# lxtGH/Video-K-Net

Hardware: AMD Instinct MI355X
Metric: frames/sec (S=3, N=100, 1024x2048) (higher is better)
Workload: dtype f32; 1 GPU; cfg2 video_knet_s3_r50: VideoKernelIterHead S=3, N=100 proposals + 17 stuff = 117 kernels, C=256, 1024x2048 frame -> 128x256 stride-8 features, ffn tracking link, x4 bilinear upsample of the final logits; streams_per_gpu=1, parallelism=frame-sharded dp1, x_storage=fp32

## Files before the change

include/vkn.h:

```cpp
#ifndef VKN_H
#define VKN_H
#include <stddef.h>
#include <stdint.h>

#ifdef __cplusplus
extern "C" {
#endif

#define VKN_VERSION 0x000600

#define VKN_OK 0
#define VKN_E_ARG (-1)
#define VKN_E_SHAPE (-2)
#define VKN_E_WORKSPACE (-3)
#define VKN_E_LAUNCH (-4)
#define VKN_E_ALIGN (-5)
#define VKN_E_RANGE (-6)

#define VKN_STATUS_RANGE 1u

#define VKN_FLAG_REF_KERNELS 1u
#define VKN_FLAG_EXACT_GEMM 2u
#define VKN_FLAG_LOGITS_HANDOFF 4u
#define VKN_FLAG_BITS_HANDOFF 16u
#define VKN_X_F32 0
#define VKN_X_F16 1
#define VKN_X_BF16 2
#define VKN_FLAG_X_F16 64u
#define VKN_FLAG_X_BF16 128u
#define VKN_FLAG_CHAIN_LAUNCHES 256u
#define VKN_FLAG_CHAIN_PERSISTENT 512u
#define VKN_FLAG_JOIN_EARLY 32768u
#define VKN_FLAG_LINK_RESERVE 262144u
#define VKN_FLAG_LINK_NO_RESERVE 524288u
#define VKN_FLAG_SCALED_F16 16384u
#define VKN_FLAG_CHAIN_BF16X3 65536u
#define VKN_FLAG_CHAIN_KSPLIT 8192u
#define VKN_FLAG_SERIAL_LINK 32u
#define VKN_FLAG_CLIP_LINK 8u

#define VKN_FLAG_INIT_SEPARATE 131072u
#define VKN_FLAG_PHASE_A 1024u
#define VKN_FLAG_PHASE_B 2048u
#define VKN_FLAG_PHASE_C 4096u
#define VKN_FLAG_PHASE_MASK (VKN_FLAG_PHASE_A | VKN_FLAG_PHASE_B | VKN_FLAG_PHASE_C)

#define VKN_MAX_FCS 4

typedef struct VknDims {
    int B;
    int N;
    int C;
    int H, W;
    int heads;
    int ff;
    int ncls;
    int n_cls_fcs, n_mask_fcs;
    float thr_logit;
    float ln_eps;
} VknDims;

typedef struct VknStageWeights {
    const float *ft_w, *ft_b, *ft_wT;
    const float *dyn_w, *dyn_b;
    const float *inp_w, *inp_b;
    const float *ig_w, *ig_b, *ug_w, *ug_b;
    const float *norm_in_w, *norm_in_b;
    const float *norm_out_w, *norm_out_b;
    const float *inorm_in_w, *inorm_in_b;
// ... 346 lines not shown
```

video-k-net_amd/csrc/vkn_api.hip:

```cpp
#include "../../include/vkn.h"
#include "../../include/vkn_decode.h"
#include "vkn_common.h"
#include "vkn_launch.h"

namespace {

struct Carver {
    char* base;
    size_t off;
    template <class T>
    T* take(size_t n) {
        off = (off + 255) & ~(size_t)255;
        T* p = base ? reinterpret_cast<T*>(base + off) : nullptr;
        off += n * sizeof(T);
        return p;
    }
};

inline bool aligned16(const void* p) { return (reinterpret_cast<uintptr_t>(p) & 15) == 0; }
inline int npt_of(int N) { return (N + 31) / 32 * 32; }

struct StageWs {
    float *part, *cntp, *xraw, *cnt, *xfeat, *params, *inputf, *ig, *ug, *f, *obj1, *qkv, *ao, *obj2, *h, *partial, *t1, *t2,
        *maskfeat, *kb, *kern32, *lq, *lkv, *lobj, *lupd, *lf;
// ... 144 lines not shown
    const int rt = (M + 31) / 32, ktiles = K / 32;
    int ks = 256 / (rt > 0 ? rt : 1);
    if (ks > 16) ks = 16;
    if (ks > ktiles) ks = ktiles;
    if (ks < 1) ks = 1;
    return ks;
}

size_t carve_stage(const VknDims* d, char* base, StageWs* s) {
    Carver c{base, 0};
    const size_t B = d->B, N = d->N, C = d->C, P = (size_t)d->H * d->W, M = B * N, FF = d->ff;
    const size_t G = vkn_gather_groups(d->B, (int)P), NPT = npt_of(d->N);
    s->status = c.take<int>(64);
    s->part = c.take<float>(B * G * NPT * C);
    s->cntp = c.take<float>(B * G * NPT);
    s->xraw = c.take<float>(M * C);
    s->cnt = c.take<float>(M);
    s->xfeat = c.take<float>(M * C);
    s->params = c.take<float>(M * 2 * C);
    s->inputf = c.take<float>(M * 2 * C);
    s->ig = c.take<float>(M * 2 * C);
    s->ug = c.take<float>(M * C);
    s->f = c.take<float>(M * C);
    s->obj1 = c.take<float>(M * C);
    s->qkv = c.take<float>(M * 3 * C);
    s->ao = c.take<float>(M * C);
    s->obj2 = c.take<float>(M * C);
    s->h = c.take<float>(M * FF);
    {
        const size_t ks = (size_t)ffn_ksplit((int)M, (int)FF), hs = (size_t)ffn_hsplit((int)M, (int)FF);
        const size_t ks1 = (size_t)ffn_ksplit((int)N, (int)FF), hs1 = (size_t)ffn_hsplit((int)N, (int)FF);
        const size_t k4 = 4;
        const size_t a = (ks > hs ? (ks > k4 ? ks : k4) : (hs > k4 ? hs : k4)) * M * C, b1 = (ks1 > hs1 ? (ks1 > k4 ? ks1 : k4) : (hs1 > k4 ? hs1 : k4)) * N * C;
        s->partial = c.take<float>(a > b1 ? a : b1);
    }
    s->t1 = c.take<float>(M * C);
    s->t2 = c.take<float>(M * C);
    s->maskfeat = c.take<float>(M * C);
    s->kb = c.take<float>(M);
    s->kern32 = c.take<float>(M * C);
    s->lq = c.take<float>(M * C);
    s->lkv = c.take<float>(M * 2 * C);
    s->lobj = c.take<float>(M * C);
    s->lupd = c.take<float>(M * C);
    s->lf = c.take<float>(M * C);
    s->kfh = c.take<_Float16>(B * NPT * C);
    s->kfl = c.take<_Float16>(B * NPT * C);
    return (c.off + 255) & ~(size_t)255;
}

int stage_ws(const VknDims* d, void* ws, size_t ws_bytes, StageWs* s) {
    if (!ws || ws_bytes < carve_stage(d, nullptr, s) || !aligned16(ws)) return VKN_E_WORKSPACE;
    carve_stage(d, static_cast<char*>(ws), s);
    return VKN_OK;
}

struct GatherWs { float *part, *cntp, *cnt; };
size_t carve_gather(int B, int N, int C, int P, char* base, GatherWs* g) {
    const size_t G = vkn_gather_groups(B, P), NPT = npt_of(N);
    Carver c{base, 0};
    g->part = c.take<float>((size_t)B * G * NPT * C);
    g->cntp = c.take<float>((size_t)B * G * NPT);
    g->cnt = c.take<float>((size_t)B * N);
    return (c.off + 255) & ~(size_t)255;
}
size_t carve_planes(int B, int N, int C, char* base, _Float16** kfh, _Float16** kfl) {
    Carver c{base, 0};
// ... 190 lines not shown
        const long long q = grid * 3 / 4;
        return (int)(q > full ? full : (q < d->B ? d->B : q));
    }
    if (mode != 1 || !persistent_chain || d->B < VKN_LINK_RESERVE_MIN_FRAMES || xdt_of(flags) != 0) return 0;
    return grid == VKN_DECODE_CUS ? full : 0;
}

inline int persistent_min_row_tiles(const PrepW& pw, unsigned flags) {
    return (!(flags & VKN_FLAG_CHAIN_BF16X3) && pw.h2_scale && pw.h2[VKN_H2_DYNFT]) ? 22 : 64;
}
inline unsigned pw_off(const VknStageWeights* w, const void* p) {
    return (unsigned)(static_cast<const char*>(p) - static_cast<const char*>(w->prepared));
}
inline bool chain_weights_ok(const PrepW& pw, bool have_cls) {
    return pw.dynft && pw.dyn && pw.dec && pw.inp && pw.ig && pw.ug && pw.fc && pw.attn_in && pw.attn_out && pw.ffn1 && pw.ffn2 &&
           pw.cls_fc[0] && pw.mask_fc[0] && (!have_cls || pw.fc_cls);
}
inline bool chain_stage_ok(const VknDims* d, const VknStageWeights* w, const PrepW& pw, bool have_cls) {
    return chain_shape_ok(d) && w->prepared && w->prepared_bytes < (1ull << 31) && chain_weights_ok(pw, have_cls) && w->ffn1_w &&
           w->cls_ln_w[0] && w->mask_ln_w[0];
}
bool chain_fast_ok(const VknDims* d, const VknStageWeights* w, const PrepW& pw, unsigned flags, bool have_cls) {
    if (flags & (VKN_FLAG_CHAIN_LAUNCHES | VKN_FLAG_EXACT_GEMM)) return false;
    if (vkn_dbg_env("VKN_CHAIN_LAUNCHES", 0)) return false;
    if (!(flags & VKN_FLAG_CHAIN_PERSISTENT) && !vkn_dbg_env("VKN_CHAIN_PERSISTENT", 0) &&
        (d->B * d->N + 31) / 32 < persistent_min_row_tiles(pw, flags))
        return false;
    return pw.chain_consts && chain_stage_ok(d, w, pw, have_cls);
}
inline bool chain_h2(const PrepW& pw, unsigned flags, bool have_cls) {
    return !(flags & VKN_FLAG_CHAIN_BF16X3) && pw.h2_scale && pw.h2[VKN_H2_DYNFT] && pw.h2[VKN_H2_DEC] && (!have_cls || pw.h2[VKN_H2_FCCLS]);
}

int run_chain_fast(const VknDims* d, const VknStageWeights* w, const PrepW& pw, const float* a0, bool a0_raw, const float* cnt,
                   const float* obj_in, float* obj_out, float* cls_logits, bool cls_sigmoid, float* kern32_out, const StageWs& s,
                   hipStream_t st, bool h2 = false) {
    const int M = d->B * d->N, C = d->C;
    VknChainA a{};
    a.a0 = a0; a.obj_in = obj_in; a.rowscale = a0_raw ? cnt : nullptr;
    a.wbase = w->prepared; a.wbytes = w->prepared_bytes;
    if (h2) {
        a.off_dyn = pw_off(w, pw.h2[a0_raw ? VKN_H2_DYNFT : VKN_H2_DYN]);
        a.off_inp = pw_off(w, pw.h2[VKN_H2_INP]); a.off_ig = pw_off(w, pw.h2[VKN_H2_IG]); a.off_ug = pw_off(w, pw.h2[VKN_H2_UG]);
        a.off_fc = pw_off(w, pw.h2[VKN_H2_FC]); a.off_in = pw_off(w, pw.h2[VKN_H2_IN]);
    } else {
        a.off_dyn = pw_off(w, a0_raw ? pw.dynft : pw.dyn);
        a.off_inp = pw_off(w, pw.inp); a.off_ig = pw_off(w, pw.ig); a.off_ug = pw_off(w, pw.ug); a.off_fc = pw_off(w, pw.fc);
        a.off_in = pw_off(w, pw.attn_in);
    }
    a.consts = pw.chain_consts;
    a.eps = d->ln_eps; a.M = M; a.obj1 = s.obj1; a.qkv = s.qkv; a.status = s.status;
    VKN_TRY(h2 ? vkn_launch_chain_a_h2(a, st) : vkn_launch_chain_a(a, st));
    VKN_TRY(vkn_launch_attn(s.qkv, 3 * C, s.qkv + C, s.qkv + 2 * C, 3 * C, s.ao, C, d->B, d->N, d->N, d->heads, C / d->heads, st));
    VknChainC c{};
    c.ao = s.ao; c.obj1 = s.obj1; c.wbase = w->prepared; c.wbytes = w->prepared_bytes;
    if (h2) {
        c.off_out = pw_off(w, pw.h2[VKN_H2_OUT]); c.off_ffn1 = pw_off(w, pw.h2[VKN_H2_FFN1]); c.off_ffn2 = pw_off(w, pw.h2[VKN_H2_FFN2]);
        c.off_clsfc = pw_off(w, pw.h2[VKN_H2_CLSFC]); c.off_maskfc = pw_off(w, pw.h2[VKN_H2_MASKFC]);
        c.off_fccls = pw.h2[VKN_H2_FCCLS] ? pw_off(w, pw.h2[VKN_H2_FCCLS]) : 0u; c.off_dec = pw_off(w, pw.h2[VKN_H2_DEC]);
    } else {
        c.off_out = pw_off(w, pw.attn_out); c.off_ffn1 = pw_off(w, pw.ffn1); c.off_ffn2 = pw_off(w, pw.ffn2);
        c.off_clsfc = pw_off(w, pw.cls_fc[0]); c.off_maskfc = pw_off(w, pw.mask_fc[0]);
        c.off_fccls = pw.fc_cls ? pw_off(w, pw.fc_cls) : 0u; c.off_dec = pw_off(w, pw.dec);
    }
    c.consts = pw.chain_consts; c.kb0 = pw.kb0;
    c.ff = d->ff; c.ncls = d->ncls; c.cls_sigmoid = cls_sigmoid ? 1 : 0; c.eps = d->ln_eps; c.M = M;
    c.obj_out = obj_out; c.cls_out = cls_logits; c.kb_out = s.kb;
    if (kern32_out) c.kern_out = kern32_out;
    else { c.plane_hi = s.kfh; c.plane_lo = s.kfl; }
    c.rows_per_frame = d->N; c.NPT = npt_of(d->N); c.status = s.status;
    return h2 ? vkn_launch_chain_c_h2(c, st) : vkn_launch_chain_c(c, st);
}

#define VKN_KS_MAX_ROW_TILES 16
inline bool ks_width_ok(const VknDims* d) {
    return chain_width_ok(d) && (d->ff % 512 == 0 || d->ff <= 1024);
}
bool chain_ks_ok(const VknDims* d, const VknStageWeights* w, const PrepW& pw, unsigned flags, bool have_cls) {
    if (flags & (VKN_FLAG_CHAIN_LAUNCHES | VKN_FLAG_CHAIN_PERSISTENT | VKN_FLAG_EXACT_GEMM)) return false;
    if (vkn_dbg_env("VKN_CHAIN_LAUNCHES", 0) || vkn_dbg_env("VKN_CHAIN_PERSISTENT", 0) || !vkn_dbg_env("VKN_CHAIN_KSPLIT", 1)) return false;
    if (!(flags & VKN_FLAG_CHAIN_KSPLIT) && (d->B * d->N + 31) / 32 > VKN_KS_MAX_ROW_TILES) return false;
    if (!ks_width_ok(d) || !chain_stage_ok(d, w, pw, have_cls)) return false;
    const void* v16[] = {w->inorm_in_w, w->inorm_in_b, w->norm_in_w, w->norm_in_b, w->norm_out_w, w->norm_out_b, w->inorm_out_w, w->inorm_out_b,
                         w->fc_norm_w, w->fc_norm_b, w->attn_norm_w, w->attn_norm_b, w->ffn_norm_w, w->ffn_norm_b, w->ffn2_b,
                         w->cls_ln_w[0], w->cls_ln_b[0], w->mask_ln_w[0], w->mask_ln_b[0], pw.dvec};
    for (const void* p : v16)
        if (!p || !aligned16(p)) return false;
    return true;
}

VknKsProb ks_prob(const float* a, int lda, const void* W, int Nout, int KT, float eps) {
    VknKsProb p{};
    p.pro.a[0] = a; p.pro.lda[0] = lda; p.pro.nsum = 1; p.pro.eps = eps;
    p.Wsplit = W; p.Nout = Nout; p.KT = KT;
    return p;
}

int run_chain_ks(const VknDims* d, const VknStageWeights* w, const PrepW& pw, const float* a0, bool a0_raw, const float* cnt,
                 const float* obj_in, float* obj_out, float* cls_logits, bool cls_sigmoid, float* kern32_out, const StageWs& s,
                 hipStream_t st, hipEvent_t obj_ready) {
    const int M = d->B * d->N, C = d->C, FF = d->ff;
    const float eps = d->ln_eps;
    VknKsProb pr[2];
    pr[0] = ks_prob(a0, C, a0_raw ? pw.dynft : pw.dyn, 2 * C, 8, eps);
// ... 146 lines not shown
                           will_fast ? w->prepared_bytes : 0));

    float* xfeat = c.x_feat_out ? c.x_feat_out : s.xfeat;
    VknEpi e = mk_epi(d);
    if (given_xfeat) {
        xfeat = const_cast<float*>(c.xfeat_in);
    } else if (has_ft) {
        if (!comp || c.x_feat_out || need_xfeat) {
            e.bias = w->ft_b; e.rowscale = s.cnt; e.out = xfeat; e.ldo = C;
            VKN_TRY(vkn_launch_gemm(s.xraw, nullptr, C, w->ft_w, pw.ft, M, C, C, 1, nullptr, e, st));
        }
    } else {
        if (hipMemcpyAsync(xfeat, s.xraw, (size_t)M * C * sizeof(float), hipMemcpyDeviceToDevice, st) != hipSuccess)
            return VKN_E_LAUNCH;
    }

    const float* obj_in = c.obj_in;
    if (pre_link) {
        PrepW pl;
        VKN_TRY(carve_pw(d, c.link_pre, flags, &pl));
        VKN_TRY(run_link(d, c.link_pre, pl, obj_in, c.prev_pre, s.lobj, s, st, c.link_pre->dyn_w ? xfeat : nullptr, flags));
        obj_in = s.lobj;
    }

    const float* kb = has_ft ? s.kb : nullptr;
    float* const kern32 = ref_decode ? (chain_only ? c.kern_out : s.kern32) : nullptr;
    const bool link = c.prev_obj && c.track_out;
    if (fast) {
        const bool raw = !given_xfeat;
        if (fewrow) {
            VKN_TRY(run_chain_ks(d, w, pw, raw ? s.xraw : xfeat, raw, s.cnt, obj_in, c.obj_out, cls_logits, c.cls_sigmoid, kern32, s, st, c.obj_ready));
        } else {
            VKN_TRY(run_chain_fast(d, w, pw, raw ? s.xraw : xfeat, raw, s.cnt, obj_in, c.obj_out, cls_logits, c.cls_sigmoid, kern32, s, st,
                                   chain_h2(pw, flags, have_cls)));
            if (c.obj_ready && hipEventRecord(c.obj_ready, st) != hipSuccess) return VKN_E_LAUNCH;
        }
        VKN_TRY(emit_masks(d, c, s, ref_decode, s.kern32, kb, touch_nx, touch_nx_bytes, flags, st, !fewrow));
        if (link) VKN_TRY(run_track_link(d, s, st, c.obj_out, c.prev_obj, c.track_out, w, c.link_track, c.track_src, xfeat, flags));
        return VKN_OK;
    }

    VKN_TRY(run_updator(d, w, pw, xfeat, (comp && !given_xfeat) ? s.xraw : nullptr, s.cnt, obj_in, s.obj1, s, st));

    VKN_TRY(run_attention(d, s, s.obj1, s.obj1, d->heads, w->attn_in_w, pw.attn_in, nullptr, w->attn_in_b, w->attn_out_w,
                          pw.attn_out, w->attn_out_b, w->attn_norm_w, w->attn_norm_b, s.obj2, st));
    if (w->ffn1_w) {
        VKN_TRY(run_ffn(d, s, s.obj2, w->ffn1_w, pw.ffn1, w->ffn1_b, w->ffn2_w, pw.ffn2, w->ffn2_b, w->ffn_norm_w,
                        w->ffn_norm_b, c.obj_out, st));
    } else {
        if (hipMemcpyAsync(c.obj_out, s.obj2, (size_t)M * C * sizeof(float), hipMemcpyDeviceToDevice, st) != hipSuccess)
            return VKN_E_LAUNCH;
    }
    const float* obj3 = c.obj_out;

    const bool fork_late = vkn_dbg_env("VKN_LINK_FORK_LATE", 0) != 0;
    if (c.obj_ready && !fork_late && hipEventRecord(c.obj_ready, st) != hipSuccess) return VKN_E_LAUNCH;

    const float* tc = obj3;
    const float* tm = obj3;
    const int nl = d->n_cls_fcs > d->n_mask_fcs ? d->n_cls_fcs : d->n_mask_fcs;
    VknGemmProb pr[2];
    for (int i = 0; i < nl; ++i) {
        int np = 0;
        if (i < d->n_cls_fcs) {
            float* dst = (i & 1) ? s.t2 : s.t1;
            e = mk_epi(d); e.ln_w = w->cls_ln_w[i]; e.ln_b = w->cls_ln_b[i]; e.act = 1; e.out = dst; e.ldo = C;
            pr[np++] = VknGemmProb{tc, nullptr, nullptr, nullptr, C, w->cls_fc_w[i], pw.cls_fc[i], C, e};
// ... 871 lines not shown
```

video-k-net_amd/csrc/vkn_chain.hip:

```cpp
#include "vkn_common.h"
#include "vkn_launch.h"

#ifdef CH_H2
typedef _Float16 ch_e;
#define CH_NPL 2
#define CH_WTILE 32768u
#define k_chain_a k_chain_a_h2
#define k_chain_c k_chain_c_h2
#define ChainAArgs ChainAArgsH2
#define ChainCArgs ChainCArgsH2
#define vkn_launch_chain_a vkn_launch_chain_a_h2
#define vkn_launch_chain_c vkn_launch_chain_c_h2
#else
typedef __bf16 ch_e;
#define CH_NPL 3
#define CH_WTILE 49152u
#endif
typedef ch_e ch_ex8 __attribute__((ext_vector_type(8)));
typedef ch_e ch_ex4 __attribute__((ext_vector_type(4)));
typedef unsigned int cu32x4 __attribute__((ext_vector_type(4)));

#define CH_THREADS 512
#define CH_ROWS 32
#define CH_C 256
// ... 358 lines not shown
        if (k < NV) *reinterpret_cast<f32x4*>(cst + 4 * k) = t[i];
    }
}

}

enum {
    CA_DYN_B = 0,
    CA_DYN_B2 = 512,
    CA_NO_W = 1024, CA_NO_B = 1280,
    CA_INP_B = 1536,
    CA_INO_W = 2048, CA_INO_B = 2304,
    CA_IG_B = 2560, CA_INI_W = 2816, CA_INI_B = 3072,
    CA_UG_B = 3328, CA_NI_W = 3584, CA_NI_B = 3840,
    CA_FC_B = 4096, CA_FCN_W = 4352, CA_FCN_B = 4608,
    CA_IN_B = 4864,
    CA_SC = 5632,
    CA_TOTAL = 5640
};

struct ChainAArgs {
    const float* a0;
    const float* obj_in;
    const float* rowscale;
    const void* wbase;
    unsigned wbytes;
    unsigned off_dyn, off_inp, off_ig, off_ug, off_fc, off_in;
    float eps;
    int M;
    float* obj1;
    float* qkv;
    const float* consts;
    int* status;
};

template <int ABL>
__global__ __launch_bounds__(CH_THREADS) void k_chain_a(const ChainAArgs A) {
    extern __shared__ __attribute__((aligned(16))) char smem_ca[];
    ch_e* IMG0 = reinterpret_cast<ch_e*>(smem_ca);
    ch_e* IMG1 = IMG0 + CH_IMG;
    float* S = reinterpret_cast<float*>(IMG1 + CH_IMG);
    float* CST = S + 2 * CH_SBUF;
    float* PARK = CST + CA_TOTAL;
#ifdef CH_H2
    float* RS = PARK + 16 * CH_THREADS;
#endif

    const int tid = threadIdx.x;
    ChLane L_ = ch_lane(tid);
    L_.status = A.status;
    const ChLane L = L_;
    const int m0 = blockIdx.x * CH_ROWS, M = A.M;
    const int row = m0 + L.li;
    const bool row_ok = row < M;
    const __amdgpu_buffer_rsrc_t wrs = __builtin_amdgcn_make_buffer_rsrc(const_cast<void*>(A.wbase), 0, (int)A.wbytes, 0x00020000);

    constexpr int RING = CH_RING_OF(ABL);
    ChRing<RING> R;
    {
        const ChNext first{A.off_dyn, A.off_dyn + 8u * CH_WTILE, 2};
#pragma unroll
        for (int j = 0; j < RING - 1; ++j) ch_wload<RING, CH_AUX_OF(ABL), CH_NP_OF(ABL)>(R, j, wrs, L, first.off(j));
        if (CH_NOLOAD(ABL)) ch_wload<RING>(R, RING - 1, wrs, L, A.off_dyn);
    }
    ch_stage_consts<CA_TOTAL>(CST, A.consts, tid);
#ifdef CH_H2
    ch_img_load(IMG0, A.a0, CH_C, m0, M, tid, RS);
    ch_img_load(IMG1, A.obj_in, CH_C, m0, M, tid, RS + 32);
#else
    ch_img_load(IMG0, A.a0, CH_C, m0, M, tid);
    ch_img_load(IMG1, A.obj_in, CH_C, m0, M, tid);
#endif
    const float bs = A.rowscale ? A.rowscale[min(row, M - 1)] : 1.f;
    CH_BAR();

    int sb = 0;
    f32x16 acc[2];
    float pout[1][16];
    ch_zero(acc[0]);
    ch_zero(acc[1]);
    ch_gemm<2, true, ABL>(acc, IMG0, IMG0, A.off_dyn, A.off_dyn + 8u * CH_WTILE, ChNext{A.off_inp, A.off_inp + 8u * CH_WTILE, 2}, R, wrs, L);
    CH_UNSCALE(acc[0], CST[CA_SC + 0] * RS[L.li]);
    CH_UNSCALE(acc[1], CST[CA_SC + 0] * RS[L.li]);
    {
        float b[16], b2[16], pin[16];
        ch_cols(CST + CA_DYN_B, L, b);
        ch_cols(CST + CA_DYN_B2, L, b2);
#pragma unroll
// ... 101 lines not shown
    CC_B2 = 768, CC_FN_W = 1024, CC_FN_B = 1280,
    CC_CLN_W = 1536, CC_CLN_B = 1792,
    CC_MLN_W = 2048, CC_MLN_B = 2304,
    CC_DVEC = 2560,
    CC_CLS_B = 2816,
    CC_DEC_B = 3072,
    CC_B1 = 3328,
    CC_SC = 3328 + 2048,
    CC_TOTAL = 3328 + 2048 + 8
};

struct ChainCArgs {
    const float* ao;
    const float* obj1;
    const void* wbase;
    unsigned wbytes;
    unsigned off_out, off_ffn1, off_ffn2, off_clsfc, off_maskfc, off_fccls, off_dec;
    int nchunks;
    int has_cls;
    int cls_sigmoid;
    int ncls;
    float eps;
    int M;
    const float* kb0;
    float* obj_out;
    float* cls_out;
    float* kb_out;
    _Float16* plane_hi;
    _Float16* plane_lo;
    float* kern_out;
    int rows_per_frame, NPT;
    const float* consts;
    int* status;
};

template <int ABL>
__global__ __launch_bounds__(CH_THREADS) void k_chain_c(const ChainCArgs A) {
    extern __shared__ __attribute__((aligned(16))) char smem_cc[];
    ch_e* IMG0 = reinterpret_cast<ch_e*>(smem_cc);
    ch_e* HID = IMG0 + CH_IMG;
    float* S = reinterpret_cast<float*>(HID + CH_IMG);
    float* CST = S + 2 * CH_SBUF;
#ifdef CH_H2
    float* RS = CST + CC_TOTAL;
#endif

    const int tid = threadIdx.x;
    ChLane L_ = ch_lane(tid);
    L_.status = A.status;
    const ChLane L = L_;
    const int m0 = blockIdx.x * CH_ROWS, M = A.M;
    const int row = m0 + L.li;
    const bool row_ok = row < M;
    const int rowc = min(row, M - 1);
    const __amdgpu_buffer_rsrc_t wrs = __builtin_amdgcn_make_buffer_rsrc(const_cast<void*>(A.wbase), 0, (int)A.wbytes, 0x00020000);

    constexpr int RING = CH_RING_OF(ABL);
    ChRing<RING> R;
    {
        const ChNext first{A.off_out, 0u, 1};
#pragma unroll
        for (int j = 0; j < RING - 1; ++j) ch_wload<RING, CH_AUX_OF(ABL), CH_NP_OF(ABL)>(R, j, wrs, L, first.off(j));
        if (CH_NOLOAD(ABL)) ch_wload<RING>(R, RING - 1, wrs, L, A.off_out);
    }
    ch_stage_consts<CC_TOTAL>(CST, A.consts, tid);
#ifdef CH_H2
    ch_img_load(IMG0, A.ao, CH_C, m0, M, tid, RS);
#else
    ch_img_load(IMG0, A.ao, CH_C, m0, M, tid);
#endif
    float obj[1][16];
    {
        const float* s = A.obj1 + (size_t)rowc * CH_C + L.wave * 32 + 4 * L.g;
#pragma unroll
        for (int q = 0; q < 4; ++q) {
            const f32x4 t = *reinterpret_cast<const f32x4*>(s + 8 * q);
#pragma unroll
            for (int e = 0; e < 4; ++e) obj[0][4 * q + e] = t[e];
        }
    }
    CH_BAR();

    int sb = 0;
    f32x16 acc1[1];
    ch_zero(acc1[0]);
    ch_gemm<1, true, ABL>(acc1, IMG0, IMG0, A.off_out, 0u, ChNext{A.off_ffn1, 0u, 1}, R, wrs, L);
    CH_UNSCALE(acc1[0], CST[CC_SC + 0] * RS[L.li]);
    {
        float b[16];
        ch_cols(CST + CC_OUT_B, L, b);
#pragma unroll
        for (int r = 0; r < 16; ++r) obj[0][r] = acc1[0][r] + b[r] + obj[0][r];
        const float* const lw[1] = {CST + CC_AN_W};
        const float* const lb[1] = {CST + CC_AN_B};
        ch_layernorm<1>(obj, lw, lb, A.eps, S, sb, L);
        ch_img_write(IMG0, obj[0], L);
        CH_BAR();
    }
    f32x16 acc2[1];
    ch_zero(acc2[0]);
#pragma unroll 1
    for (int c = 0; c < A.nchunks; ++c) {
        ch_zero(acc1[0]);
        ch_gemm<1, true, ABL>(acc1, IMG0, IMG0, A.off_ffn1 + (unsigned)c * 8u * CH_WTILE, 0u,
                         ChNext{A.off_ffn2 + (unsigned)c * 8u * CH_WTILE, 0u, 1}, R, wrs, L);
        CH_UNSCALE(acc1[0], CST[CC_SC + 1]);
        float h[16], b[16];
        ch_cols(CST + CC_B1 + 256 * c, L, b);
#pragma unroll
        for (int r = 0; r < 16; ++r) h[r] = fmaxf(acc1[0][r] + b[r], 0.f);
        CH_BAR();
        ch_img_write(HID, h, L);
        CH_BAR();
        const bool lastc = (c + 1 == A.nchunks);
        const ChNext nx = lastc ? ChNext{A.off_clsfc, A.off_maskfc, 2} : ChNext{A.off_ffn1 + (unsigned)(c + 1) * 8u * CH_WTILE, 0u, 1};
        ch_gemm<1, true, ABL>(acc2, HID, HID, A.off_ffn2 + (unsigned)c * 8u * CH_WTILE, 0u, nx, R, wrs, L);
    }
    CH_UNSCALE(acc2[0], CST[CC_SC + 2]);
    {
        float b[16];
        ch_cols(CST + CC_B2, L, b);
#pragma unroll
        for (int r = 0; r < 16; ++r) obj[0][r] = obj[0][r] + acc2[0][r] + b[r];
        const float* const lw[1] = {CST + CC_FN_W};
        const float* const lb[1] = {CST + CC_FN_B};
        ch_layernorm<1>(obj, lw, lb, A.eps, S, sb, L);
        ch_store_rows(A.obj_out, CH_C, 0, row, row_ok, obj[0], L);
        ch_img_write(IMG0, obj[0], L);
        CH_BAR();
    }
    f32x16 acc[2];
    ch_zero(acc[0]);
    ch_zero(acc[1]);
    const ChNext nfin = A.has_cls ? ChNext{A.off_fccls, A.off_dec, 2} : ChNext{A.off_dec, 0u, 1};
    ch_gemm<2, true, ABL>(acc, IMG0, IMG0, A.off_clsfc, A.off_maskfc, nfin, R, wrs, L);
    CH_UNSCALE(acc[0], CST[CC_SC + 3]);
    CH_UNSCALE(acc[1], CST[CC_SC + 4]);
    {
        float t[2][16];
#pragma unroll
        for (int r = 0; r < 16; ++r) {
            t[0][r] = acc[0][r];
            t[1][r] = acc[1][r];
        }
        const float* const lw[2] = {CST + CC_CLN_W, CST + CC_MLN_W};
        const float* const lb[2] = {CST + CC_CLN_B, CST + CC_MLN_B};
        ch_layernorm<2>(t, lw, lb, A.eps, S, sb, L);
        float dv[16], kd[1];
        ch_cols(CST + CC_DVEC, L, dv);
// ... 343 lines not shown

#else
__global__ __launch_bounds__(256) void k_split_h2(const float* __restrict__ W, _Float16* __restrict__ Wp, int Nout, int K,
                                                  const float* __restrict__ scale) {
    const int kt = blockIdx.x, nt = blockIdx.y;
    _Float16* dst = Wp + ((size_t)nt * gridDim.x + kt) * (CH_WTILE / 2);
    const int row = threadIdx.x, n = nt * 256 + row;
    const float sc = scale[0];
    for (int k = 0; k < 32; ++k) {
        ch_e t[2] = {(ch_e)0.f, (ch_e)0.f};
        if (n < Nout) ch_split(W[(size_t)n * K + kt * 32 + k] * sc, t);
        const int q = k >> 3, e = k & 7;
        dst[((0 * 4 + q) * 256 + row) * 8 + e] = t[0];
        dst[((1 * 4 + q) * 256 + row) * 8 + e] = t[1];
    }
}
size_t vkn_split_h2_bytes(int Nout, int K) { return (size_t)((Nout + 255) / 256) * (size_t)(K / 32) * CH_WTILE; }
int vkn_launch_split_h2(const float* W, void* images, int Nout, int K, const float* scale, hipStream_t stream) {
    if (!W || !images || !scale || Nout <= 0 || K <= 0 || K % 32 != 0) return VKN_E_ARG;
    hipLaunchKernelGGL(k_split_h2, dim3(K / 32, (Nout + 255) / 256), dim3(256), 0, stream, W, static_cast<_Float16*>(images), Nout, K, scale);
    VKN_CHECK_LAUNCH();
    return VKN_OK;
}
#endif

int vkn_launch_chain_a(const VknChainA& p, hipStream_t stream) {
    if (!p.a0 || !p.obj_in || !p.wbase || !p.obj1 || !p.qkv || !p.consts || p.M <= 0 || p.wbytes >= (1ull << 31)) return VKN_E_ARG;
    ChainAArgs A{};
    A.a0 = p.a0; A.obj_in = p.obj_in; A.rowscale = p.rowscale; A.wbase = p.wbase; A.wbytes = (unsigned)p.wbytes;
    A.off_dyn = p.off_dyn; A.off_inp = p.off_inp; A.off_ig = p.off_ig; A.off_ug = p.off_ug; A.off_fc = p.off_fc; A.off_in = p.off_in;
    A.eps = p.eps; A.M = p.M; A.obj1 = p.obj1; A.qkv = p.qkv;
    A.consts = p.consts + (p.rowscale ? 0 : CA_TOTAL);
    A.status = p.status;
#ifdef CH_H2
    const size_t lds = (size_t)2 * CH_IMG * sizeof(ch_e) + (size_t)(2 * CH_SBUF + CA_TOTAL + 16 * CH_THREADS + 64 + 512) * sizeof(float);
#else
    const size_t lds = (size_t)2 * CH_IMG * sizeof(ch_e) + (size_t)(2 * CH_SBUF + CA_TOTAL + 16 * CH_THREADS) * sizeof(float);
#endif
#define CHA_LAUNCH(ABLV)                                                                                            \
    do {                                                                                                            \
        VKN_ALLOW_FULL_LDS(k_chain_a<ABLV>);                                                                        \
        hipLaunchKernelGGL(k_chain_a<ABLV>, dim3((p.M + CH_ROWS - 1) / CH_ROWS), dim3(CH_THREADS), lds, stream, A); \
    } while (0)
#ifdef VKN_DEBUG
    switch (vkn_dbg_env("VKN_CHAIN_ABL", 0)) {
        case 1: CHA_LAUNCH(1); break;
        case 2: CHA_LAUNCH(2); break;
        case 3: CHA_LAUNCH(3); break;
        case 4: CHA_LAUNCH(4); break;
        case 5: CHA_LAUNCH(5); break;
        case 6: CHA_LAUNCH(6); break;
        case 7: CHA_LAUNCH(7); break;
        case 8: CHA_LAUNCH(8); break;
        case 9: CHA_LAUNCH(9); break;
        case 10: CHA_LAUNCH(10); break;
        case 11: CHA_LAUNCH(11); break;
        default: CHA_LAUNCH(0); break;
    }
#else
    CHA_LAUNCH(0);
#endif
#undef CHA_LAUNCH
    VKN_CHECK_LAUNCH();
    return VKN_OK;
}

int vkn_launch_chain_c(const VknChainC& p, hipStream_t stream) {
    if (!p.ao || !p.obj1 || !p.wbase || !p.obj_out || !p.consts || p.M <= 0 || p.wbytes >= (1ull << 31)) return VKN_E_ARG;
    if (p.ff <= 0 || p.ff % 256 != 0 || p.ff > 2048 || p.ncls > 256) return VKN_E_SHAPE;
    if (!p.plane_hi == !p.kern_out || (p.plane_hi && !p.plane_lo)) return VKN_E_ARG;
    ChainCArgs A{};
    A.ao = p.ao; A.obj1 = p.obj1; A.wbase = p.wbase; A.wbytes = (unsigned)p.wbytes;
    A.off_out = p.off_out; A.off_ffn1 = p.off_ffn1; A.off_ffn2 = p.off_ffn2; A.off_clsfc = p.off_clsfc; A.off_maskfc = p.off_maskfc;
    A.off_fccls = p.off_fccls; A.off_dec = p.off_dec;
    A.nchunks = p.ff / 256; A.has_cls = (p.cls_out != nullptr) ? 1 : 0; A.cls_sigmoid = p.cls_sigmoid; A.ncls = p.ncls;
    A.eps = p.eps; A.M = p.M; A.kb0 = p.kb0; A.obj_out = p.obj_out; A.cls_out = p.cls_out; A.kb_out = p.kb_out;
    A.plane_hi = p.plane_hi; A.plane_lo = p.plane_lo; A.kern_out = p.kern_out; A.rows_per_frame = p.rows_per_frame; A.NPT = p.NPT;
    A.consts = p.consts + 2 * CA_TOTAL;
    A.status = p.status;
#ifdef CH_H2
    const size_t lds = (size_t)2 * CH_IMG * sizeof(ch_e) + (size_t)(2 * CH_SBUF + CC_TOTAL + 32) * sizeof(float);
#else
    const size_t lds = (size_t)2 * CH_IMG * sizeof(ch_e) + (size_t)(2 * CH_SBUF + CC_TOTAL) * sizeof(float);
#endif
#define CHC_LAUNCH(ABLV)                                                                                            \
    do {                                                                                                            \
        VKN_ALLOW_FULL_LDS(k_chain_c<ABLV>);                                                                        \
        hipLaunchKernelGGL(k_chain_c<ABLV>, dim3((p.M + CH_ROWS - 1) / CH_ROWS), dim3(CH_THREADS), lds, stream, A); \
    } while (0)
#ifdef VKN_DEBUG
    switch (vkn_dbg_env("VKN_CHAIN_ABL", 0)) {
        case 1: CHC_LAUNCH(1); break;
        case 2: CHC_LAUNCH(2); break;
        case 3: CHC_LAUNCH(3); break;
        case 4: CHC_LAUNCH(4); break;
        case 5: CHC_LAUNCH(5); break;
        case 6: CHC_LAUNCH(6); break;
        case 7: CHC_LAUNCH(7); break;
        case 8: CHC_LAUNCH(8); break;
        case 9: CHC_LAUNCH(9); break;
        case 10: CHC_LAUNCH(10); break;
        case 11: CHC_LAUNCH(11); break;
        default: CHC_LAUNCH(0); break;
    }
#else
    CHC_LAUNCH(0);
#endif
#undef CHC_LAUNCH
    VKN_CHECK_LAUNCH();
    return VKN_OK;
}
```

video-k-net_amd/csrc/vkn_launch.h:

```cpp
#pragma once
#include <hip/hip_runtime.h>
#include <stddef.h>

struct VknEpi {
    const float* bias;
    const float* rowscale;
    const float* bias2;
    const float* resid;
    int ldr;
    const float* ln_w;
    const float* ln_b;
    int ln_from_col;
    float eps;
    int act;
    float* out;
    int ldo;
    const float* dot_vec;
    const float* dot_bias;
    float* dot_out;
    _Float16* plane_hi;
    _Float16* plane_lo;
    int rows_per_frame;
    int NPT;
};
// ... 93 lines not shown

struct VknPanopticCfg;
size_t vkn_panoptic_ws_bytes(int B, int K, int Ho, int Wo);
int vkn_launch_panoptic_joint(const VknPanopticCfg* c, const float* cls, const float* masks, int B, int N, int ncls,
                              int* panoptic_seg, int* info, int* nseg, int* bbox, void* ws, size_t ws_bytes, hipStream_t st);

struct VknChainConsts {
    const float *bcnt, *dyn_b;
    const float *norm_out_w, *norm_out_b, *inp_b, *inorm_out_w, *inorm_out_b;
    const float *ig_b, *inorm_in_w, *inorm_in_b, *ug_b, *norm_in_w, *norm_in_b;
    const float *fc_b, *fc_norm_w, *fc_norm_b, *in_b;
    const float *out_b, *attn_norm_w, *attn_norm_b, *ffn1_b, *ffn2_b, *ffn_norm_w, *ffn_norm_b;
    const float *cls_ln_w, *cls_ln_b, *mask_ln_w, *mask_ln_b, *dvec, *fc_cls_b, *dec_b;
    int ff, ncls;
    const float* h2_inv[14];
};
enum { VKN_H2_DYNFT = 0, VKN_H2_DYN, VKN_H2_INP, VKN_H2_IG, VKN_H2_UG, VKN_H2_FC, VKN_H2_IN, VKN_H2_OUT, VKN_H2_FFN1, VKN_H2_FFN2,
       VKN_H2_CLSFC, VKN_H2_MASKFC, VKN_H2_FCCLS, VKN_H2_DEC, VKN_H2_COUNT };
size_t vkn_chain_consts_floats();
int vkn_chain_pack_consts(const VknChainConsts& c, float* out, hipStream_t stream);
struct VknChainA {
    const float* a0;
    const float* obj_in;
    const float* rowscale;
    const void* wbase;
    size_t wbytes;
    unsigned off_dyn, off_inp, off_ig, off_ug, off_fc, off_in;
    const float* consts;
    float eps;
    int M;
    float* obj1;
    float* qkv;
    int* status;
};
struct VknChainC {
    const float* ao;
    const float* obj1;
    const void* wbase;
    size_t wbytes;
    unsigned off_out, off_ffn1, off_ffn2, off_clsfc, off_maskfc, off_fccls, off_dec;
    const float* consts;
    const float* kb0;
    int ff, ncls, cls_sigmoid;
    float eps;
    int M;
    float* obj_out;
    float* cls_out;
    float* kb_out;
    _Float16 *plane_hi, *plane_lo;
    float* kern_out;
    int rows_per_frame, NPT;
    int* status;
};
int vkn_launch_gemm_t3(const VknGemmProb* probs, int nprob, int M, int K, hipStream_t stream);
int vkn_launch_chain_a(const VknChainA& p, hipStream_t stream);
int vkn_launch_chain_c(const VknChainC& p, hipStream_t stream);
int vkn_launch_chain_a_h2(const VknChainA& p, hipStream_t stream);
int vkn_launch_chain_c_h2(const VknChainC& p, hipStream_t stream);
size_t vkn_split_h2_bytes(int Nout, int K);
int vkn_launch_split_h2(const float* W, void* images, int Nout, int K, const float* scale, hipStream_t stream);

struct VknKsPro {
    const float* a[4];
    int lda[4];
    int nsum;
    long long sum_stride;
    const float* pbias;
    const float* presid;
    int ldr;
    const float* ln_w[4];
    const float* ln_b[4];
    float eps;
    int act;
    float* side_out;
    int ld_side;
    const float* dot_vec;
    const float* dot_bias;
    float* dot_out;
};
struct VknKsEpi {
    const float* bias;
    const float* rowscale;
    const float* bias2;
    const float* resid;
    int ldr;
    int act;
// ... 16 lines not shown
```

video-k-net_amd/ops.py:

```python
import contextlib
import ctypes
import struct
import threading

import torch

from . import _lib
from ._lib import VknDims, VknStageWeights, check

_H = _lib.CONSTS
FLAG_REF_KERNELS = _H['VKN_FLAG_REF_KERNELS']
FLAG_EXACT_GEMM = _H['VKN_FLAG_EXACT_GEMM']
FLAG_LOGITS_HANDOFF = _H['VKN_FLAG_LOGITS_HANDOFF']
FLAG_BITS_HANDOFF = _H['VKN_FLAG_BITS_HANDOFF']
FLAG_CHAIN_LAUNCHES = _H['VKN_FLAG_CHAIN_LAUNCHES']
FLAG_CHAIN_PERSISTENT = _H['VKN_FLAG_CHAIN_PERSISTENT']
FLAG_JOIN_EARLY = _H['VKN_FLAG_JOIN_EARLY']
FLAG_LINK_RESERVE = _H['VKN_FLAG_LINK_RESERVE']
FLAG_LINK_NO_RESERVE = _H['VKN_FLAG_LINK_NO_RESERVE']
FLAG_SCALED_F16 = _H['VKN_FLAG_SCALED_F16']
FLAG_CHAIN_BF16X3 = _H['VKN_FLAG_CHAIN_BF16X3']
FLAG_INIT_SEPARATE = _H['VKN_FLAG_INIT_SEPARATE']
FLAG_CHAIN_KSPLIT = _H['VKN_FLAG_CHAIN_KSPLIT']
FLAG_SERIAL_LINK = _H['VKN_FLAG_SERIAL_LINK']

_tls = threading.local()


def _ptr(t):
    return ctypes.c_void_p(t.data_ptr()) if t is not None else ctypes.c_void_p(0)


def _stream():
    return ctypes.c_void_p(torch.cuda.current_stream().cuda_stream)


def _req(t, name):
    if not torch.is_tensor(t) or not t.is_cuda:
        raise _lib.VknLibraryError(f'{name}: expected a CUDA/HIP tensor — the MI355X path has no CPU fallback')
    if t.dtype != torch.float32:
        raise TypeError(f'{name}: expected float32, got {t.dtype}')
    t = t.contiguous()
    if t.data_ptr() % 16:
        t = t.clone(memory_format=torch.contiguous_format)
    return t


_X_DTYPES = {torch.float32: _H['VKN_X_F32'], torch.float16: _H['VKN_X_F16'], torch.bfloat16: _H['VKN_X_BF16']}
FLAG_X_F16, FLAG_X_BF16 = _H['VKN_FLAG_X_F16'], _H['VKN_FLAG_X_BF16']


def _req_x(t, name='x'):
    if not torch.is_tensor(t) or not t.is_cuda:
        raise _lib.VknLibraryError(f'{name}: expected a CUDA/HIP tensor — the MI355X path has no CPU fallback')
    if t.dtype not in _X_DTYPES:
# ... 1659 lines not shown
```

Baseline: 10070 frames/s.

## Split chain-C FFN hidden dimension across workgroups with ticketed partial-sum reduction

Splits the FFN hidden chunks of the fused chain-C kernel across 2 or 4 workgroups per row tile. Each workgroup writes its FFN2 partial accumulators to global scratch, and the last arriving workgroup (tracked with an atomic ticket) sums the partials and runs the epilogue. Chain-A zeroes the tickets, and blocks can be strided so a tile's split workgroups land on the same XCD. The goal is more parallelism for the small row count (M=117 gives only 4 tiles), at the cost of extra global traffic, atomics and duplicated attn-out/FFN1 prologue work.

```diff
diff --git a/include/vkn.h b/include/vkn.h
--- a/include/vkn.h
+++ b/include/vkn.h
@@ -35,6 +35,8 @@
 #define VKN_FLAG_LINK_NO_RESERVE 524288u
 #define VKN_FLAG_SCALED_F16 16384u
 #define VKN_FLAG_CHAIN_BF16X3 65536u
+#define VKN_FLAG_CHAIN_FFN_SPLIT 1048576u
+#define VKN_FLAG_CHAIN_NO_FFN_SPLIT 2097152u
 #define VKN_FLAG_CHAIN_KSPLIT 8192u
 #define VKN_FLAG_SERIAL_LINK 32u
 #define VKN_FLAG_CLIP_LINK 8u
diff --git a/video-k-net_amd/csrc/vkn_api.hip b/video-k-net_amd/csrc/vkn_api.hip
--- a/video-k-net_amd/csrc/vkn_api.hip
+++ b/video-k-net_amd/csrc/vkn_api.hip
@@ -200,7 +200,9 @@
         const size_t ks1 = (size_t)ffn_ksplit((int)N, (int)FF), hs1 = (size_t)ffn_hsplit((int)N, (int)FF);
         const size_t k4 = 4;
         const size_t a = (ks > hs ? (ks > k4 ? ks : k4) : (hs > k4 ? hs : k4)) * M * C, b1 = (ks1 > hs1 ? (ks1 > k4 ? ks1 : k4) : (hs1 > k4 ? hs1 : k4)) * N * C;
-        s->partial = c.take<float>(a > b1 ? a : b1);
+        const size_t sp = C == 256 ? vkn_chain_split_floats(M) : 0, sp1 = C == 256 ? vkn_chain_split_floats(N) : 0;
+        const size_t ab = a > b1 ? a : b1, sps = sp > sp1 ? sp : sp1;
+        s->partial = c.take<float>(ab > sps ? ab : sps);
     }
     s->t1 = c.take<float>(M * C);
     s->t2 = c.take<float>(M * C);
@@ -457,11 +459,27 @@
     return !(flags & VKN_FLAG_CHAIN_BF16X3) && pw.h2_scale && pw.h2[VKN_H2_DYNFT] && pw.h2[VKN_H2_DEC] && (!have_cls || pw.h2[VKN_H2_FCCLS]);
 }
 
+#define VKN_CHAIN_SPLIT_MAX_WGS 232
+inline int chain_c_hsplit(const VknDims* d, unsigned flags, bool h2) {
+    if (!h2 || (flags & VKN_FLAG_CHAIN_NO_FFN_SPLIT) || d->ff % 256 != 0) return 1;
+    const int nch = d->ff / 256, G = nch < 4 ? nch : 4, rt = (d->B * d->N + 31) / 32;
+    if (G < 2 || (G & 1) || nch % G != 0) return 1;
+    const int dbg = vkn_dbg_env("VKN_CHAIN_SPLIT_HS", 0);
+    if (dbg == 1 || ((dbg == 2 || dbg == 4) && G % dbg == 0)) return dbg;
+    const int L = vkn_dbg_env("VKN_CHAIN_SPLIT_L", VKN_CHAIN_SPLIT_MAX_WGS);
+    if (G == 4 && 4 * rt <= L) return 4;
+    if (2 * rt <= L || (flags & VKN_FLAG_CHAIN_FFN_SPLIT)) return 2;
+    return 1;
+}
+
 int run_chain_fast(const VknDims* d, const VknStageWeights* w, const PrepW& pw, const float* a0, bool a0_raw, const float* cnt,
                    const float* obj_in, float* obj_out, float* cls_logits, bool cls_sigmoid, float* kern32_out, const StageWs& s,
-                   hipStream_t st, bool h2 = false) {
+                   hipStream_t st, bool h2 = false, unsigned flags = 0) {
     const int M = d->B * d->N, C = d->C;
+    const int hs = chain_c_hsplit(d, flags, h2);
+    unsigned* const tickets = hs > 1 ? vkn_chain_split_tickets(s.partial, (size_t)M) : nullptr;
     VknChainA a{};
+    a.tickets = tickets;
     a.a0 = a0; a.obj_in = obj_in; a.rowscale = a0_raw ? cnt : nullptr;
     a.wbase = w->prepared; a.wbytes = w->prepared_bytes;
     if (h2) {
@@ -494,7 +512,9 @@
     if (kern32_out) c.kern_out = kern32_out;
     else { c.plane_hi = s.kfh; c.plane_lo = s.kfl; }
     c.rows_per_frame = d->N; c.NPT = npt_of(d->N); c.status = s.status;
-    return h2 ? vkn_launch_chain_c_h2(c, st) : vkn_launch_chain_c(c, st);
+    c.hs = hs; c.ffn_part = hs > 1 ? s.partial : nullptr; c.tickets = tickets;
+    c.same_xcd = vkn_dbg_env("VKN_CHAIN_SPLIT_XCD", 1);
+    return h2 ?vkn_launch_chain_c_h2(c, st) : vkn_launch_chain_c(c, st);
 }
 
 #define VKN_KS_MAX_ROW_TILES 16
@@ -707,7 +727,7 @@
             VKN_TRY(run_chain_ks(d, w, pw, raw ? s.xraw : xfeat, raw, s.cnt, obj_in, c.obj_out, cls_logits, c.cls_sigmoid, kern32, s, st, c.obj_ready));
         } else {
             VKN_TRY(run_chain_fast(d, w, pw, raw ? s.xraw : xfeat, raw, s.cnt, obj_in, c.obj_out, cls_logits, c.cls_sigmoid, kern32, s, st,
-                                   chain_h2(pw, flags, have_cls)));
+                                   chain_h2(pw, flags, have_cls), flags));
             if (c.obj_ready && hipEventRecord(c.obj_ready, st) != hipSuccess) return VKN_E_LAUNCH;
         }
         VKN_TRY(emit_masks(d, c, s, ref_decode, s.kern32, kb, touch_nx, touch_nx_bytes, flags, st, !fewrow));
diff --git a/video-k-net_amd/csrc/vkn_chain.hip b/video-k-net_amd/csrc/vkn_chain.hip
--- a/video-k-net_amd/csrc/vkn_chain.hip
+++ b/video-k-net_amd/csrc/vkn_chain.hip
@@ -414,6 +414,7 @@
     float* qkv;
     const float* consts;
     int* status;
+    unsigned* tickets;
 };
 
 template <int ABL>
@@ -436,6 +437,7 @@
     const int row = m0 + L.li;
     const bool row_ok = row < M;
     const __amdgpu_buffer_rsrc_t wrs = __builtin_amdgcn_make_buffer_rsrc(const_cast<void*>(A.wbase), 0, (int)A.wbytes, 0x00020000);
+    if (A.tickets && tid == 0) A.tickets[blockIdx.x] = 0u;
 
     constexpr int RING = CH_RING_OF(ABL);
     ChRing<RING> R;
@@ -603,9 +605,13 @@
     int rows_per_frame, NPT;
     const float* consts;
     int* status;
+    float* part;
+    unsigned* tickets;
+    int ntiles;
+    int xcd_stride;
 };
 
-template <int ABL>
+template <int ABL, int HS>
 __global__ __launch_bounds__(CH_THREADS) void k_chain_c(const ChainCArgs A) {
     extern __shared__ __attribute__((aligned(16))) char smem_cc[];
     ch_e* IMG0 = reinterpret_cast<ch_e*>(smem_cc);
@@ -614,13 +620,30 @@
     float* CST = S + 2 * CH_SBUF;
 #ifdef CH_H2
     float* RS = CST + CC_TOTAL;
+    unsigned* TK = reinterpret_cast<unsigned*>(RS + 32);
+#else
+    unsigned* TK = reinterpret_cast<unsigned*>(CST + CC_TOTAL);
 #endif
 
     const int tid = threadIdx.x;
     ChLane L_ = ch_lane(tid);
     L_.status = A.status;
     const ChLane L = L_;
-    const int m0 = blockIdx.x * CH_ROWS, M = A.M;
+    int tile = blockIdx.x, wpart = 0;
+    if constexpr (HS > 1) {
+        if (A.xcd_stride) {
+            wpart = (int)blockIdx.x / A.xcd_stride;
+            tile = (int)blockIdx.x - wpart * A.xcd_stride;
+            if (tile >= A.ntiles) return;
+        } else {
+            tile = (int)blockIdx.x / HS;
+            wpart = (int)blockIdx.x - tile * HS;
+        }
+    }
+    const int G = A.nchunks < 4 ? A.nchunks : 4, cpg = (HS > 1) ? A.nchunks / G : 1;
+    const int c0 = (HS > 1) ? wpart * (G / HS) * cpg : 0, c1 = (HS > 1) ? c0 + (G / HS) * cpg : A.nchunks;
+    const __amdgpu_buffer_rsrc_t prs = __builtin_amdgcn_make_buffer_rsrc(A.part, 0, HS > 1 ? A.ntiles * G * (CH_ROWS * CH_C * 4) : 0, 0x00020000);
+    const int m0 = tile * CH_ROWS, M = A.M;
     const int row = m0 + L.li;
     const bool row_ok = row < M;
     const int rowc = min(row, M - 1);
@@ -655,7 +678,7 @@
     int sb = 0;
     f32x16 acc1[1];
     ch_zero(acc1[0]);
-    ch_gemm<1, true, ABL>(acc1, IMG0, IMG0, A.off_out, 0u, ChNext{A.off_ffn1, 0u, 1}, R, wrs, L);
+    ch_gemm<1, true, ABL>(acc1, IMG0, IMG0, A.off_out, 0u, ChNext{A.off_ffn1 + (unsigned)c0 * 8u * CH_WTILE, 0u, 1}, R, wrs, L);
     CH_UNSCALE(acc1[0], CST[CC_SC + 0] * RS[L.li]);
     {
         float b[16];
@@ -671,7 +694,10 @@
     f32x16 acc2[1];
     ch_zero(acc2[0]);
 #pragma unroll 1
-    for (int c = 0; c < A.nchunks; ++c) {
+    for (int c = c0; c < c1; ++c) {
+        if constexpr (HS > 1) {
+            if ((c & (cpg - 1)) == 0) ch_zero(acc2[0]);
+        }
         ch_zero(acc1[0]);
         ch_gemm<1, true, ABL>(acc1, IMG0, IMG0, A.off_ffn1 + (unsigned)c * 8u * CH_WTILE, 0u,
                          ChNext{A.off_ffn2 + (unsigned)c * 8u * CH_WTILE, 0u, 1}, R, wrs, L);
@@ -683,9 +709,42 @@
         CH_BAR();
         ch_img_write(HID, h, L);
         CH_BAR();
-        const bool lastc = (c + 1 == A.nchunks);
+        const bool lastc = (c + 1 == c1);
         const ChNext nx = lastc ? ChNext{A.off_clsfc, A.off_maskfc, 2} : ChNext{A.off_ffn1 + (unsigned)(c + 1) * 8u * CH_WTILE, 0u, 1};
         ch_gemm<1, true, ABL>(acc2, HID, HID, A.off_ffn2 + (unsigned)c * 8u * CH_WTILE, 0u, nx, R, wrs, L);
+        if constexpr (HS > 1) {
+            if (((c + 1) & (cpg - 1)) == 0) {
+                const int po = (tile * G + c / cpg) * (CH_ROWS * CH_C * 4);
+#pragma unroll
+                for (int q = 0; q < 4; ++q)
+                    __builtin_amdgcn_raw_buffer_store_b128(__builtin_bit_cast(cu32x4, f32x4{acc2[0][4 * q], acc2[0][4 * q + 1], acc2[0][4 * q + 2], acc2[0][4 * q + 3]}),
+                                                           prs, (q * CH_THREADS + tid) * 16, po, 16);
+            }
+        }
+    }
+    if constexpr (HS > 1) {
+        asm volatile("s_waitcnt vmcnt(0)" ::: "memory");
+        __syncthreads();
+        if (tid == 0) {
+            const unsigned t = __hip_atomic_fetch_add(A.tickets + tile, 1u, __ATOMIC_RELAXED, __HIP_MEMORY_SCOPE_AGENT);
+            if (t == (unsigned)(HS - 1)) {
+                __builtin_amdgcn_fence(__ATOMIC_ACQUIRE, "agent");
+                asm volatile("s_waitcnt vmcnt(0)" ::: "memory");
+            }
+            *TK = t;
+        }
+        __syncthreads();
+        if (*TK != (unsigned)(HS - 1)) return;
+#pragma unroll 1
+        for (int g = 0; g < G; ++g) {
+            const int po = (tile * G + g) * (CH_ROWS * CH_C * 4);
+#pragma unroll
+            for (int q = 0; q < 4; ++q) {
+                const f32x4 t = __builtin_bit_cast(f32x4, __builtin_amdgcn_raw_buffer_load_b128(prs, (q * CH_THREADS + tid) * 16, po, 16));
+#pragma unroll
+                for (int e = 0; e < 4; ++e) acc2[0][4 * q + e] = (g == 0) ? t[e] : acc2[0][4 * q + e] + t[e];
+            }
+        }
     }
     CH_UNSCALE(acc2[0], CST[CC_SC + 2]);
     {
@@ -1095,6 +1154,7 @@
     A.eps = p.eps; A.M = p.M; A.obj1 = p.obj1; A.qkv = p.qkv;
     A.consts = p.consts + (p.rowscale ? 0 : CA_TOTAL);
     A.status = p.status;
+    A.tickets = p.tickets;
 #ifdef CH_H2
     const size_t lds = (size_t)2 * CH_IMG * sizeof(ch_e) + (size_t)(2 * CH_SBUF + CA_TOTAL + 16 * CH_THREADS + 64 + 512) * sizeof(float);
 #else
@@ -1132,6 +1192,13 @@
     if (!p.ao || !p.obj1 || !p.wbase || !p.obj_out || !p.consts || p.M <= 0 || p.wbytes >= (1ull << 31)) return VKN_E_ARG;
     if (p.ff <= 0 || p.ff % 256 != 0 || p.ff > 2048 || p.ncls > 256) return VKN_E_SHAPE;
     if (!p.plane_hi == !p.kern_out || (p.plane_hi && !p.plane_lo)) return VKN_E_ARG;
+    const int hs = p.hs > 1 ? p.hs : 1, ntiles = (p.M + CH_ROWS - 1) / CH_ROWS;
+    if (hs > 1) {
+        const int nch = p.ff / 256, G = nch < 4 ? nch : 4;
+        if ((hs != 2 && hs != 4) || nch % G != 0 || G % hs != 0) return VKN_E_SHAPE;
+        if (!p.ffn_part || !p.tickets || (reinterpret_cast<uintptr_t>(p.ffn_part) & 15)) return VKN_E_ARG;
+        if ((size_t)ntiles * 4 * CH_ROWS * CH_C * 4 >= (1ull << 31)) return VKN_E_SHAPE;
+    }
     ChainCArgs A{};
     A.ao = p.ao; A.obj1 = p.obj1; A.wbase = p.wbase; A.wbytes = (unsigned)p.wbytes;
     A.off_out = p.off_out; A.off_ffn1 = p.off_ffn1; A.off_ffn2 = p.off_ffn2; A.off_clsfc = p.off_clsfc; A.off_maskfc = p.off_maskfc;
@@ -1141,16 +1208,23 @@
     A.plane_hi = p.plane_hi; A.plane_lo = p.plane_lo; A.kern_out = p.kern_out; A.rows_per_frame = p.rows_per_frame; A.NPT = p.NPT;
     A.consts = p.consts + 2 * CA_TOTAL;
     A.status = p.status;
-#ifdef CH_H2
-    const size_t lds = (size_t)2 * CH_IMG * sizeof(ch_e) + (size_t)(2 * CH_SBUF + CC_TOTAL + 32) * sizeof(float);
-#else
-    const size_t lds = (size_t)2 * CH_IMG * sizeof(ch_e) + (size_t)(2 * CH_SBUF + CC_TOTAL) * sizeof(float);
-#endif
-#define CHC_LAUNCH(ABLV)                                                                                            \
+    A.part = p.ffn_part; A.tickets = p.tickets; A.ntiles = ntiles;
+    A.xcd_stride = (hs > 1 && p.same_xcd) ? (ntiles + 7) / 8 * 8 : 0;
+    const int nblocks = hs == 1 ? ntiles : (A.xcd_stride ? hs * A.xcd_stride : hs * ntiles);
+#ifdef CH_H2
+    const size_t lds = (size_t)2 * CH_IMG * sizeof(ch_e) + (size_t)(2 * CH_SBUF + CC_TOTAL + 32 + (hs > 1 ? 4 : 0)) * sizeof(float);
+#else
+    const size_t lds = (size_t)2 * CH_IMG * sizeof(ch_e) + (size_t)(2 * CH_SBUF + CC_TOTAL + (hs > 1 ? 4 : 0)) * sizeof(float);
+#endif
+#define CHC_LAUNCH_HS(ABLV, HSV)                                                                                    \
     do {                                                                                                            \
-        VKN_ALLOW_FULL_LDS(k_chain_c<ABLV>);                                                                        \
-        hipLaunchKernelGGL(k_chain_c<ABLV>, dim3((p.M + CH_ROWS - 1) / CH_ROWS), dim3(CH_THREADS), lds, stream, A); \
+        VKN_ALLOW_FULL_LDS((k_chain_c<ABLV, HSV>));                                                                 \
+        hipLaunchKernelGGL((k_chain_c<ABLV, HSV>), dim3(nblocks), dim3(CH_THREADS), lds, stream, A);                \
     } while (0)
+#define CHC_LAUNCH(ABLV) CHC_LAUNCH_HS(ABLV, 1)
+    if (hs == 4) CHC_LAUNCH_HS(0, 4);
+    else if (hs == 2) CHC_LAUNCH_HS(0, 2);
+    else
 #ifdef VKN_DEBUG
     switch (vkn_dbg_env("VKN_CHAIN_ABL", 0)) {
         case 1: CHC_LAUNCH(1); break;
@@ -1170,6 +1244,7 @@
     CHC_LAUNCH(0);
 #endif
 #undef CHC_LAUNCH
+#undef CHC_LAUNCH_HS
     VKN_CHECK_LAUNCH();
     return VKN_OK;
 }
diff --git a/video-k-net_amd/csrc/vkn_launch.h b/video-k-net_amd/csrc/vkn_launch.h
--- a/video-k-net_amd/csrc/vkn_launch.h
+++ b/video-k-net_amd/csrc/vkn_launch.h
@@ -149,6 +149,7 @@
     float* obj1;
     float* qkv;
     int* status;
+    unsigned* tickets;
 };
 struct VknChainC {
     const float* ao;
@@ -168,7 +169,18 @@
     float* kern_out;
     int rows_per_frame, NPT;
     int* status;
-};
+    int hs;
+    float* ffn_part;
+    unsigned* tickets;
+    int same_xcd;
+};
+inline size_t vkn_chain_split_floats(size_t M) {
+    const size_t rt = (M + 31) / 32;
+    return rt * 4 * 32 * 256 + (rt + 63) / 64 * 64;
+}
+inline unsigned* vkn_chain_split_tickets(float* ffn_part, size_t M) {
+    return reinterpret_cast<unsigned*>(ffn_part + (M + 31) / 32 * 4 * 32 * 256);
+}
 int vkn_launch_gemm_t3(const VknGemmProb* probs, int nprob, int M, int K, hipStream_t stream);
 int vkn_launch_chain_a(const VknChainA& p, hipStream_t stream);
 int vkn_launch_chain_c(const VknChainC& p, hipStream_t stream);
diff --git a/video-k-net_amd/ops.py b/video-k-net_amd/ops.py
--- a/video-k-net_amd/ops.py
+++ b/video-k-net_amd/ops.py
@@ -20,7 +20,9 @@
 FLAG_LINK_NO_RESERVE = _H['VKN_FLAG_LINK_NO_RESERVE']
 FLAG_SCALED_F16 = _H['VKN_FLAG_SCALED_F16']
 FLAG_CHAIN_BF16X3 = _H['VKN_FLAG_CHAIN_BF16X3']
-FLAG_INIT_SEPARATE = _H['VKN_FLAG_INIT_SEPARATE']
+FLAG_CHAIN_FFN_SPLIT = _H['VKN_FLAG_CHAIN_FFN_SPLIT']
+FLAG_CHAIN_NO_FFN_SPLIT = _H['VKN_FLAG_CHAIN_NO_FFN_SPLIT']
+FLAG_INIT_SEPARATE =_H['VKN_FLAG_INIT_SEPARATE']
 FLAG_CHAIN_KSPLIT = _H['VKN_FLAG_CHAIN_KSPLIT']
 FLAG_SERIAL_LINK = _H['VKN_FLAG_SERIAL_LINK']
 
```

Result: no change. 10050 frames/s (median of 2 runs) (-0.2%).
